# hamaadshah/gan_deeplearning4j

Measured on NVIDIA H100. Metric: images/sec (full G+D step), higher is better.
Workload: dtype bf16

## Files before the change

gan_deeplearning4j_b200/_lib.py:

```python
from __future__ import annotations

import ctypes as C
import os

_HERE = os.path.dirname(os.path.abspath(__file__))
LIB_PATH = os.path.join(_HERE, "lib", "libb200gan.so")
NAME_LEN = 64


class B200GanError(RuntimeError):
    def __init__(self, code, msg):
        super().__init__(f"libb200gan error {code}: {msg}")
        self.code = code


class LayerDesc(C.Structure):
    _fields_ = [("type", C.c_int32), ("name", C.c_char * NAME_LEN), ("n_in", C.c_int32), ("n_out", C.c_int32),
                ("k_h", C.c_int32), ("k_w", C.c_int32), ("s_h", C.c_int32), ("s_w", C.c_int32), ("p_h", C.c_int32), ("p_w", C.c_int32),
                ("has_bias", C.c_int32), ("act", C.c_int32), ("act_alpha", C.c_float), ("updater", C.c_int32),
                ("lr", C.c_float), ("beta1", C.c_float), ("beta2", C.c_float), ("eps", C.c_float), ("l2", C.c_float),
                ("bn_decay", C.c_float), ("bn_eps", C.c_float), ("pre_h", C.c_int32), ("pre_w", C.c_int32), ("pre_c", C.c_int32),
                ("loss", C.c_int32), ("frozen", C.c_int32)]


# ... 25 lines not shown
    _fields_ = [("l1", C.c_float), ("l2", C.c_float), ("l1_bias", C.c_float), ("l2_bias", C.c_float)]


class Constraint(C.Structure):
    _fields_ = [("kind", C.c_int32), ("dims_mask", C.c_int32), ("max_norm", C.c_double), ("min_norm", C.c_double), ("rate", C.c_double)]


class ConvGeom(C.Structure):
    _fields_ = [(k, C.c_int32) for k in ("n", "h", "w", "c", "oh", "ow", "o", "kh", "kw", "sh", "sw", "ph", "pw")]


class TestConvOpts(C.Structure):
    _fields_ = [("epi", C.c_int32), ("act", C.c_int32), ("alpha", C.c_float), ("bias", C.POINTER(C.c_float)), ("scale", C.POINTER(C.c_float)),
                ("groups", C.c_int32), ("aux", C.POINTER(C.c_float)), ("aux2", C.POINTER(C.c_float)), ("stats", C.POINTER(C.c_double)), ("kernel", C.c_char * 64),
                ("bn", C.c_int32), ("max_ctas", C.c_int32), ("poison", C.c_int32), ("w_mn", C.c_int32), ("per_tap", C.c_int32), ("slab", C.c_int32),
                ("defer", C.c_int32), ("db", C.POINTER(C.c_float)), ("param_offset", C.c_int32), ("splits", C.c_int32)]


class EwReduceJob(C.Structure):
    _fields_ = [("n", C.c_int64), ("stride", C.c_int64), ("src_off", C.c_int64), ("dst_off", C.c_int64), ("splits", C.c_int32), ("wide", C.c_int32)]


class TestEwOpts(C.Structure):
    _fields_ = [("op", C.c_int32), ("n", C.c_int64), ("rows", C.c_int32), ("cols", C.c_int32), ("groups", C.c_int32), ("splits", C.c_int32),
                ("stride", C.c_int64)] + [(k, C.c_int32) for k in ("N", "H", "W", "C", "KH", "KW", "SH", "SW", "act")] + [
                ("alpha", C.c_float), ("clip_eps", C.c_float), ("offset", C.c_int32), ("in_place", C.c_int32), ("accumulate", C.c_int32),
                ("poison", C.c_int32), ("n_jobs", C.c_int32), ("jobs", C.POINTER(EwReduceJob)), ("n_seg", C.c_int32),
                ("seg_off", C.POINTER(C.c_int64)), ("seg_len", C.POINTER(C.c_int64)), ("seg_coef", C.POINTER(C.c_float)), ("sumsq", C.c_double),
                ("kernel", C.c_char * 64), ("loss", C.c_int32)]


# ... 107 lines not shown
```

gan_deeplearning4j_b200/csrc/engine.cu:

```cuda
#include <cuda_runtime.h>
#include <dlfcn.h>
#include <math.h>
#include <stdarg.h>
#include <stdio.h>
#include <stdlib.h>
#include <string.h>

#include <algorithm>
#include <string>
#include <vector>

#include "../../include/b200gan.h"
#include "kernels.h"

using namespace b2g;

static thread_local char g_err[1024] = "";
static int32_t fail(int32_t code, const char* fmt, ...) {
  va_list ap; va_start(ap, fmt); vsnprintf(g_err, sizeof(g_err), fmt, ap); va_end(ap); return code;
}
#define CU(call) do { cudaError_t e_ = (call); if (e_ != cudaSuccess) return fail(B2G_ERR_CUDA, "%s:%d %s -> %s", __FILE__, __LINE__, #call, cudaGetErrorString(e_)); } while (0)
#define B2(call) do { int32_t r_ = (call); if (r_ != 0) return r_; } while (0)
#define CHECK_KERNELS() CU(cudaGetLastError())

// ... 1900 lines not shown
    if (!h || prec == PREC_F32) return downF(h, (const float*)d, count);
    float* f = nullptr; B2(upF(nullptr, count, &f)); k_nhwc_to_nchw_f32(prec, d, f, 1, 1, (int)count, s); return downF(h, f, count); }
  int32_t event(cudaEvent_t* e) { CU(cudaEventCreate(e)); events.push_back(*e); return 0; }
};
}

extern "C" int32_t b2g_ctx_allreduce_test(b2g_ctx* c, float* host, int64_t n) {
  if (!c || !host || n < 1) return fail(B2G_ERR_ARG, "null"); if (!c->comm) return fail(B2G_ERR_NCCL, "no communicator"); CU(cudaSetDevice(c->device));
  HookMem m(c->stream, PREC_F32); float* d = nullptr;
  B2(m.upF(host, (size_t)n, &d));
  NC(g_nccl.ar(d, d, (size_t)n, 7, 0, c->comm, c->stream));
  B2(m.downF(host, d, (size_t)n)); CU(cudaStreamSynchronize(c->stream)); return 0;
}

struct TcTestSchedule {
  TcTestSchedule(int bn, int max_ctas, int per_tap, int splits) { g_tc_test_bn = bn; g_tc_test_max_ctas = max_ctas; g_tc_test_per_tap = per_tap; g_tc_test_splits = splits; }
  ~TcTestSchedule() { reset(); }
  void reset() { g_tc_test_bn = 0; g_tc_test_max_ctas = 0; g_tc_test_per_tap = 0; g_tc_test_splits = 0; }
};
enum : unsigned { CO_STATS = 1u << EPI_STATS, CO_BNBWD = 1u << EPI_BNBWD, CO_ACTBWD = 1u << EPI_ACTBWD, CO_BIAS_ACT = 1u << 4, CO_SCALE = 1u << 5,
                  CO_POFF = 1u << 6, CO_BN = 1u << 7, CO_MAX_CTAS = 1u << 8, CO_PER_TAP = 1u << 9, CO_W_MN = 1u << 10, CO_SPLITS = 1u << 11,
                  CO_DEFER = 1u << 12, CO_DB = 1u << 13 };
struct ConvHookImpl {
  const char* kernel;
  bool bf16, tma;
  struct { bool (*shape)(const ConvGeom&); unsigned opts; } kind[3];
};
static bool any_shape(const ConvGeom&) { return true; }
static bool dense_bwd_shape(const ConvGeom& g) { return dense_small_o_supported(g) || dense_small_k_supported(g); }
static bool tc_edge_conv_shape(const ConvGeom& g) { return edge_conv_small_cin_supported(g) && tc_edge_conv_supported(g); }
static bool tc_edge_wgrad_shape(const ConvGeom& g) { return edge_wgrad_small_cin_supported(g) && tc_edge_wgrad_supported(g); }
static const unsigned CO_TC = CO_STATS | CO_BNBWD | CO_ACTBWD | CO_BIAS_ACT | CO_SCALE | CO_BN | CO_MAX_CTAS | CO_PER_TAP;
static const ConvHookImpl kConvHook[6] = {
  {"SIMT kernel", false, false, {{any_shape, CO_BIAS_ACT | CO_SCALE | CO_POFF}, {any_shape, CO_BIAS_ACT | CO_SCALE | CO_POFF}, {any_shape, CO_POFF}}},
  {"tensor-core kernel (BF16, a working tensor-map encoder)", true, true,
   {{tc_fprop_supported, CO_TC | CO_W_MN}, {tc_dgrad_supported, CO_TC}, {tc_wgrad_supported, CO_POFF | CO_SPLITS | CO_DEFER}}},
  {"skinny-layer kernel (<= 4 image channels)", false, false,
   {{edge_conv_small_cin_supported, CO_BIAS_ACT | CO_POFF}, {edge_deconv_small_c_supported, CO_BIAS_ACT | CO_POFF}, {edge_wgrad_small_cin_supported, CO_POFF}}},
  {"skinny-layer tensor-core kernel (BF16, <= 4 image channels, a working tensor-map encoder)", true, true,
   {{tc_edge_conv_shape, CO_BIAS_ACT | CO_MAX_CTAS}, {tc_deconv_ps_supported, CO_ACTBWD | CO_BIAS_ACT | CO_MAX_CTAS},
    {tc_edge_wgrad_shape, CO_POFF | CO_SPLITS | CO_DEFER | CO_DB}}},
  {"dense kernel (1x1 geometry: <= 4 output units, or a short reduction in the input / weight gradient)", false, false,
   {{dense_small_o_supported, CO_BIAS_ACT | CO_POFF}, {dense_bwd_shape, CO_BIAS_ACT | CO_POFF}, {dense_bwd_shape, CO_POFF}}},
  {"few-output conv kernel (BF16, O <= 4, C % 8 == 0, k x k)", true, false,
   {{head_conv_supported, CO_BIAS_ACT | CO_POFF}, {head_conv_supported, CO_BIAS_ACT | CO_POFF}, {head_conv_supported, CO_POFF | CO_SPLITS | CO_DB}}},
};
static constexpr int ik(int impl, int kind) { return 3 * impl + kind; }
// ... 13 lines not shown
    return fail(B2G_ERR_UNSUPPORTED, "impl %d kind %d: no %s for this shape", impl, kind, im.kernel);
  const b2g_test_conv_opts none{}; const b2g_test_conv_opts& o = opt ? *opt : none;
  const struct { unsigned flag; bool set; const char* what; } asked[] = {
    {o.epi >= EPI_STATS && o.epi <= EPI_ACTBWD ? 1u << o.epi : 1u, o.epi != 0,
     "fused epilogue (epi 1-3: the tensor-core fprop / dgrad, impl 1 kind 0 / 1; epi 3: the pixel-shuffle deconv, impl 3 kind 1)"},
    {CO_BIAS_ACT, o.bias || o.act, "bias / activation (kinds 0 / 1; impl 4 kind 1 on its short-reduction kernel)"},
    {CO_SCALE, o.scale != nullptr, "scale (the SIMT and tensor-core fprop / dgrad, impl 0 / 1 kind 0 / 1)"},
    {CO_POFF, o.param_offset != 0, "param_offset (impl 0 / 2 / 4 / 5, and the tensor-core weight gradients, impl 1 / 3 kind 2)"},
    {CO_BN, o.bn != 0, "bn (the tile width of the tensor-core fprop / dgrad, impl 1 kind 0 / 1)"},
    {CO_MAX_CTAS, o.max_ctas != 0, "max_ctas (a grid cap of tc_conv_kernel and tc_edge_conv_kernel launches, impl 1 / 3 kind 0 / 1)"},
    {CO_PER_TAP, o.per_tap != 0, "per_tap (the tensor-core fprop / dgrad, impl 1 kind 0 / 1)"},
    {CO_W_MN, o.w_mn != 0, "w_mn (the [C][O] weight operand of the 1x1 tensor-core fprop, impl 1 kind 0)"},
    {CO_SPLITS, o.splits != 0, "splits (a forced split count of the weight gradients of impl 1 / 3 / 5)"},
    {CO_DEFER, o.defer != 0, "defer (the tensor-core weight gradients, impl 1 / 3 kind 2)"},
    {CO_DB, o.db != nullptr, "db (the bias column of the edge tensor-core and few-output weight gradients, impl 3 / 5 kind 2)"},
  };
  for (const auto& a : asked) if (a.set && !(im.kind[kind].opts & a.flag)) return fail(B2G_ERR_UNSUPPORTED, "impl %d kind %d takes no %s", impl, kind, a.what);
  if (o.param_offset < 0 || o.max_ctas < 0 || o.splits < 0)
    return fail(B2G_ERR_UNSUPPORTED, "param_offset %d, max_ctas %d, splits %d: none may be negative", o.param_offset, o.max_ctas, o.splits);
  if (o.bn && ((o.bn != 64 && o.bn != 128) || oc % o.bn))
    return fail(B2G_ERR_UNSUPPORTED, "bn %d: the tensor-core fprop / dgrad tile is 64 or 128 columns and must divide the %d output channels", o.bn, oc);
  if (impl == 4 && kind == 1 && (o.bias || o.act) && !dense_small_k_supported(g))
    return fail(B2G_ERR_UNSUPPORTED, "impl 4 kind 1: bias / activation run on the short-reduction kernel only, which has no variant for this shape");
  if (o.w_mn && (g.KH != 1 || g.KW != 1)) return fail(B2G_ERR_UNSUPPORTED, "w_mn: the [C][O] weight operand exists for the 1x1 tensor-core fprop only");
  const bool gemm = impl == 0 || impl == 2 || impl >= 4, tc_wg = kind == 2 && (impl == 1 || impl == 3);
  const int force_splits = o.splits;
  size_t sc = std::max(std::max(std::max(k_simt_wgrad_scratch_floats(g), k_tc_wgrad_scratch_floats(g)), std::max(k_edge_wgrad_scratch_floats(g), k_tc_edge_wgrad_scratch_floats(g))), k_dense_small_o_wgrad_scratch_floats(g)) + 16;
  if (force_splits) sc = std::max(sc, (size_t)force_splits * (impl == 1 || impl == 5 ? nw : (size_t)64 * 16 * g.C + 64) + 16);
  if (impl == 5) sc = std::max(sc, std::max(k_head_wgrad_scratch_floats(g), k_colsum_scratch_floats(g.O)) + 16);
  const size_t woff = (prec == PREC_F32 && kind != 2) ? (size_t)o.param_offset : 0, dwoff = kind == 2 ? (size_t)o.param_offset : 0;
// ... 10 lines not shown
  epi.mode = o.epi; epi.scale = scale; epi.imgs_per_group = g.N / groups; epi.act = act; epi.alpha = alpha;
  if (o.epi == EPI_STATS || o.epi == EPI_BNBWD) { B2(m.dev(k_bn_acc_elems(oc, groups), 8, (void**)&d_acc)); epi.acc = d_acc; }
  if (o.epi == EPI_BNBWD || o.epi == EPI_ACTBWD) {
    if (!o.aux) return fail(B2G_ERR_ARG, "epilogue %d needs aux", o.epi);
    void* aux = nullptr; B2(m.upT(o.aux, no, &aux)); epi.aux = (const __nv_bfloat16*)aux;
  }
  if (o.epi == EPI_BNBWD) {
    if (!o.aux2) return fail(B2G_ERR_ARG, "epilogue 2 needs aux2 (the BatchNorm input z)");
    void* aux2 = nullptr; B2(m.upT(o.aux2, no, &aux2)); epi.aux2 = (const __nv_bfloat16*)aux2;
  }
  const TcEpi* pe = o.epi || o.scale ? &epi : nullptr;
  const __nv_bfloat16 *ba = (const __nv_bfloat16*)ta, *bb = (const __nv_bfloat16*)tb; __nv_bfloat16* bo = (__nv_bfloat16*)to;
  ReduceList rl{}; ReduceList* prl = o.defer ? &rl : nullptr;
  cudaEvent_t e0, e1; B2(m.event(&e0)); B2(m.event(&e1));
  int reps = iters < 1 ? 1 : iters; int rc = 0, db_written = 0;
  g_tc_last_kernel = ""; g_tc_last_slab = false; g_tc_last_splits = 0; g_gemm_last_kernel = ""; g_gemm_last_splits = 0;
  TcTestSchedule schedule(o.bn, o.max_ctas, o.per_tap != 0, force_splits);
  for (int it = -1; it < reps; ++it) {
    if (it == 0) CU(cudaEventRecord(e0, s));
    if (d_acc) CU(cudaMemsetAsync(d_acc, 0, 8 * k_bn_acc_elems(oc, groups), s));
    if (o.poison) CU(cudaMemsetAsync(to, 0xFF, ts * no, s));
    if (o.poison && kind == 2) { CU(cudaMemsetAsync(fres, 0xFF, 4 * no, s)); CU(cudaMemsetAsync(scratch, 0xFF, 4 * sc, s)); }
    if (o.poison && dbres) CU(cudaMemsetAsync(dbres, 0xFF, 4 * (size_t)g.O, s));
    switch (ik(impl, kind)) {
      case ik(0, 0): k_simt_fprop(prec, prec, g, ta, tb, bias, to, act, alpha, s, scale); break;
      case ik(0, 1): k_simt_dgrad(prec, prec, g, ta, tb, bias, to, act, alpha, s, scale); break;
      case ik(0, 2): k_simt_wgrad(prec, g, ta, tb, fres, scratch, sc, 0, s); break;
      case ik(1, 0): rc = k_tc_fprop(g, ba, bb, bias, bo, act, alpha, s, pe, o.w_mn ? 1 : 0); break;
      case ik(1, 1): rc = k_tc_dgrad(g, ba, bb, bias, bo, act, alpha, s, pe); break;
      case ik(1, 2): rc = k_tc_wgrad(g, ba, bb, fres, scratch, sc, 0, s, prl); break;
      case ik(2, 0): k_edge_conv_small_cin(prec, prec, g, ta, tb, bias, to, act, alpha, s); break;
      case ik(2, 1): k_edge_deconv_small_c(prec, prec, g, ta, tb, bias, to, act, alpha, s); break;
// ... 19 lines not shown
    }
    if (rc) break;
    if (o.defer) {
      if (!rl.count) { rc = -4; break; }
      k_reduce_multi(rl, s); rl.count = 0;
    }
  }
  schedule.reset();
  CU(cudaEventRecord(e1, s));
  if (rc == -4) return fail(B2G_ERR_CUDA, "defer: the weight gradient queued no reduction");
  if (rc == -5) return fail(B2G_ERR_ARG, "splits %d: the partials do not fit the scratch", force_splits);
  if (rc) return fail(B2G_ERR_CUDA, "tensor-core kernel launch failed (%d)", rc);
  if (opt) {
    strncpy(opt->kernel, gemm ? g_gemm_last_kernel : g_tc_last_kernel, sizeof(opt->kernel) - 1); opt->kernel[sizeof(opt->kernel) - 1] = 0; opt->slab = g_tc_last_slab;
    opt->splits = gemm ? g_gemm_last_splits : tc_wg ? g_tc_last_splits : 0;
  }
  if (o.db) {
    if (!db_written) return fail(B2G_ERR_UNSUPPORTED, "the edge weight gradient produces no bias column for C = %d", g.C);
    B2(m.downF(o.db, dbres, g.O));
  }
  B2(kind == 2 ? m.downF(out, fres, no) : m.downT(out, to, no));
  CU(cudaStreamSynchronize(s)); CHECK_KERNELS();
  if (d_acc && o.stats) {
    std::vector<long long> h(k_bn_acc_elems(oc, groups)); CU(cudaMemcpy(h.data(), d_acc, 8 * h.size(), cudaMemcpyDeviceToHost));
    for (int gi = 0; gi < groups; ++gi) for (int st = 0; st < 2; ++st) for (int ch = 0; ch < oc; ++ch)
      o.stats[((size_t)gi * 2 + st) * oc + ch] = (double)h[((size_t)(gi * 2 + st) * 2 + 0) * oc + ch] / 1024.0 + (double)h[((size_t)(gi * 2 + st) * 2 + 1) * oc + ch] / 1152921504606846976.0;
  }
  float ms = 0.f; CU(cudaEventElapsedTime(&ms, e0, e1)); if (ms_per_iter) *ms_per_iter = ms / reps;
  return 0;
}
// ... 445 lines not shown
```

gan_deeplearning4j_b200/csrc/kernels.h:

```cpp
#pragma once
#include <cuda_runtime.h>
#include <cuda_bf16.h>
#include <math.h>
#include <stdint.h>

namespace b2g {

enum Prec { PREC_F32 = 0, PREC_BF16 = 1 };
enum Act { ACT_IDENTITY = 0, ACT_TANH = 1, ACT_SIGMOID = 2, ACT_RELU = 3, ACT_LRELU = 4,
           ACT_ELU = 5, ACT_SELU = 6, ACT_SOFTPLUS = 7, ACT_SOFTSIGN = 8, ACT_HARDTANH = 9, ACT_HARDSIGMOID = 10, ACT_RELU6 = 11, ACT_SWISH = 12,
           ACT_CUBE = 13, ACT_RATIONALTANH = 14, ACT_RECTIFIEDTANH = 15, ACT_THRESHOLDEDRELU = 16, ACT_EXT_FIRST = ACT_ELU, ACT_EXT_LAST = ACT_THRESHOLDEDRELU };
enum Loss { LOSS_MSE = 2, LOSS_L1 = 3, LOSS_L2 = 4, LOSS_MAE = 5, LOSS_HINGE = 6, LOSS_SQUARED_HINGE = 7, LOSS_WASSERSTEIN = 8 };

inline size_t prec_size(int prec) { return prec == PREC_F32 ? 4 : 2; }

struct ConvGeom {
  int N, H, W, C;
  int OH, OW, O;
  int KH, KW, SH, SW, PH, PW;
};

extern uint64_t g_launch_count;
extern const char* g_ew_last_kernel;
int device_sm_count();
// ... 222 lines not shown
bool head_conv_supported(const ConvGeom& g);
size_t k_head_wgrad_scratch_floats(const ConvGeom& g);
void k_head_fwd(const ConvGeom& g, const __nv_bfloat16* x, const __nv_bfloat16* w, const float* bias, __nv_bfloat16* out, int act, float alpha, cudaStream_t s);
void k_head_dgrad(const ConvGeom& g, const __nv_bfloat16* dy, const __nv_bfloat16* w, const float* bias, __nv_bfloat16* dx, int act, float alpha, cudaStream_t s);
int k_head_wgrad(const ConvGeom& g, const __nv_bfloat16* x, const __nv_bfloat16* dy, float* dw, float* part, size_t part_floats, int force_splits, cudaStream_t s,
                 ReduceList* defer);

bool tc_fprop_supported(const ConvGeom& g);
bool tc_dgrad_supported(const ConvGeom& g);
bool tc_wgrad_supported(const ConvGeom& g);
int  tc_init();
extern const char* g_tc_last_kernel;
extern int g_tc_test_bn, g_tc_test_max_ctas;
extern int g_tc_test_per_tap;
extern bool g_tc_last_slab;
extern int g_tc_test_splits, g_tc_last_splits;
enum { EPI_PLAIN = 0, EPI_STATS = 1, EPI_BNBWD = 2, EPI_ACTBWD = 3 };
struct TcEpi {
  int mode;
  const float* scale;
  unsigned long long* acc;
  int imgs_per_group;
  const __nv_bfloat16* aux;
  const __nv_bfloat16* aux2;
  int act; float alpha;
};
int k_tc_fprop(const ConvGeom& g, const __nv_bfloat16* x, const __nv_bfloat16* w, const float* bias, __nv_bfloat16* out, int act, float alpha, cudaStream_t s, const TcEpi* epi = nullptr, int w_mn = 0);
int k_tc_dgrad(const ConvGeom& g, const __nv_bfloat16* dy, const __nv_bfloat16* w, const float* bias, __nv_bfloat16* dx, int act, float alpha, cudaStream_t s, const TcEpi* epi = nullptr);
int k_tc_wgrad(const ConvGeom& g, const __nv_bfloat16* x, const __nv_bfloat16* dy, float* dw, float* scratch, size_t scratch_floats, int accumulate, cudaStream_t s, ReduceList* defer = nullptr);
size_t k_tc_wgrad_scratch_floats(const ConvGeom& g);
// ... 13 lines not shown
```

gan_deeplearning4j_b200/csrc/kernels_tc.cu:

```cuda
#include <cuda.h>
#include <stdio.h>
#include <stdlib.h>
#include <algorithm>

#include "common.cuh"
#include "kernels.h"

namespace b2g {

typedef CUresult (*PFN_encodeTiled)(CUtensorMap*, CUtensorMapDataType, cuuint32_t, void*, const cuuint64_t*, const cuuint64_t*, const cuuint32_t*,
                                    const cuuint32_t*, CUtensorMapInterleave, CUtensorMapSwizzle, CUtensorMapL2promotion, CUtensorMapFloatOOBfill);
static PFN_encodeTiled g_encode = nullptr;

int tc_init() {
  if (g_encode) return 0;
  void* fn = nullptr; cudaDriverEntryPointQueryResult q;
  if (cudaGetDriverEntryPoint("cuTensorMapEncodeTiled", &fn, cudaEnableDefault, &q) != cudaSuccess || !fn || q != cudaDriverEntryPointSuccess) return -1;
  g_encode = (PFN_encodeTiled)fn; return 0;
}

static int make_map_bf16(CUtensorMap* m, const void* base, int rank, const cuuint64_t* dims, const cuuint64_t* strides_bytes, const cuuint32_t* box, const cuuint32_t* estr) {
  if (!g_encode) return -1;
  CUresult r = g_encode(m, CU_TENSOR_MAP_DATA_TYPE_BFLOAT16, (cuuint32_t)rank, const_cast<void*>(base), dims, strides_bytes, box, estr, CU_TENSOR_MAP_INTERLEAVE_NONE,
                        CU_TENSOR_MAP_SWIZZLE_128B, CU_TENSOR_MAP_L2_PROMOTION_L2_256B, CU_TENSOR_MAP_FLOAT_OOB_FILL_NONE);
// ... 251 lines not shown
        const float s = ((sst[(0 * 2 + st) * BN + col] + sst[(1 * 2 + st) * BN + col]) + sst[(2 * 2 + st) * BN + col]) + sst[(3 * 2 + st) * BN + col];
        sacc_add(p.acc + (size_t)(group * 2 + st) * 2 * p.OC, (size_t)p.OC, (size_t)(nb0 + col), s);
      }
    }
  }
}

template <int BN>
__device__ __forceinline__ void load_b_tile(const TcConvParams& p, const CUtensorMap* tmB, uint32_t dst, uint32_t bar, int ch, int wtap, int nb0) {
  if (!p.b_mn) tma_load_3d(dst, tmB, bar, ch * 64, wtap, nb0);
  else {
#pragma unroll
    for (int j = 0; j < (BN >= 64 ? BN / 64 : 1); ++j) tma_load_3d(dst + j * 8192, tmB, bar, nb0 + j * 64, wtap, ch * 64);
  }
}
template <int BN, int NB, int NACC>
__device__ __forceinline__ void mma_kblock(float (&acc)[NB][NACC], uint32_t a_smem, uint32_t b_smem, int b_mn) {
  const uint64_t adesc = desc_kmajor_sw128(a_smem);
  if constexpr (BN < 64) {
    const uint64_t bdesc = desc_kmajor_sw128(b_smem);
#pragma unroll
    for (int k = 0; k < 4; ++k) wgmma_n16(acc[0], adesc + 2 * k, bdesc + 2 * k);
  } else if constexpr (NB == 2) {
    if (!b_mn) {
#pragma unroll
      for (int k = 0; k < 4; ++k) wgmma_n128<0, 0>(acc[0], acc[1], adesc + 2 * k, desc_kmajor_sw128(b_smem) + 2 * k);
    } else {
#pragma unroll
      for (int k = 0; k < 4; ++k) wgmma_n128<0, 1>(acc[0], acc[1], adesc + 2 * k, desc_mnmajor_sw128(b_smem + k * 2048, 8192));
    }
// ... 7 lines not shown
}
__device__ __forceinline__ void tap_coords(const TcConvParams& p, int ta, int tb, int py, int px, int& ax, int& dy_, int& wtap) {
  if (p.mode == 0) { dy_ = -p.PH + ta; ax = -p.PW + tb; wtap = ta * p.KW + tb; }
  else {
    const int r = py == 0 ? (ta == 0 ? 1 : 3) : (ta == 0 ? 0 : 2), dyr = py == 0 ? (ta == 0 ? 0 : -1) : (ta == 0 ? 1 : 0);
    const int sx = px == 0 ? (tb == 0 ? 1 : 3) : (tb == 0 ? 0 : 2), dxc = px == 0 ? (tb == 0 ? 0 : -1) : (tb == 0 ? 1 : 0);
    dy_ = dyr; ax = dxc; wtap = r * 4 + sx;
  }
}
__device__ __forceinline__ void slab_coords(const TcConvParams& p, int ta, int tb, int py, int px, int& ax, int& dy_, int& wlo, int& whi) {
  int ax2, dy2;
  tap_coords(p, p.mode == 0 ? ta : 1, tb, py, px, ax, dy_, wlo);
  tap_coords(p, p.mode == 0 ? ta + 2 : 0, tb, py, px, ax2, dy2, whi);
}

template <int BN>
struct TcConvRegs {
  static constexpr int LAUNCH = 96, PRODUCER = 24, MMA = BN >= 128 ? 96 : 64, EPI = BN >= 128 ? 128 : 160;
  static_assert(PRODUCER + 2 * MMA + 2 * EPI <= 5 * LAUNCH, "setmaxnreg budget exceeds the launch allocation");
};
template <int BN, int STAGES, int EPI, bool AFFINE, bool PS = false, bool SLAB = false>
__global__ void __launch_bounds__(TC_CONV_THREADS, 1) tc_conv_kernel(const __grid_constant__ CUtensorMap tmA, const __grid_constant__ CUtensorMap tmB, const TcConvParams p) {
  using S = TcSmem<BN, STAGES, EPI, SLAB>;
  using R = TcConvRegs<BN>;
  constexpr int NB = BN >= 64 ? BN / 64 : 1, NACC = BN >= 64 ? 32 : BN / 2;
  extern __shared__ uint8_t smem_raw[];
  const uint32_t smem_base = (smem_u32(smem_raw) + 1023u) & ~1023u;
  uint8_t* smem_gen = smem_raw + (smem_base - smem_u32(smem_raw));
  const uint32_t bar_full = smem_base + S::BAR_OFF;
  const uint32_t bar_empty = bar_full + 8 * STAGES;
  const uint32_t park_full = bar_empty + 8 * STAGES;
  const uint32_t park_empty = park_full + 8 * S::PARKS;
  float* sst = reinterpret_cast<float*>(smem_gen + S::STAT_OFF);
  const int warp = threadIdx.x >> 5, lane = threadIdx.x & 31;
  const int num_kb = p.taps_h * p.taps_w * p.chunks;
  const int tiles = p.tiles_m * p.tiles_n * p.phases;
  auto tile_coords = [&](int t, int& nb0, int& phase, int& n0, int& y0) {
    const int mt = t % p.tiles_m, r = t / p.tiles_m;
    nb0 = (r % p.tiles_n) * BN; phase = r / p.tiles_n;
    if (p.Nt > 1) { n0 = mt * p.Nt; y0 = 0; } else { n0 = mt / p.tiles_y; y0 = (mt % p.tiles_y) * p.Ht; }
  };

  if (threadIdx.x == 0) {
    prefetch_map(&tmA); prefetch_map(&tmB);
    for (int s = 0; s < STAGES; ++s) { mbar_init(bar_full + 8 * s, 1); mbar_init(bar_empty + 8 * s, 8); }
    for (int k = 0; k < S::PARKS; ++k) { mbar_init(park_full + 8 * k, 256); mbar_init(park_empty + 8 * k, 256); }
    fence_mbar_init();
  }
  __syncthreads();
  pdl_wait();

  if (warp >= 16) {
    setmaxnreg_dec<R::PRODUCER>();
    if (warp == 16) {
      int s = 0; uint32_t ph = 0;
      for (int t = blockIdx.x; t < tiles; t += gridDim.x) {
        int nb0, phase, n0, y0; tile_coords(t, nb0, phase, n0, y0);
        const int py = phase >> 1, px = phase & 1;
        const int ybase = p.mode == 0 ? y0 * p.SH : y0;
        int ch = 0, ta = 0, tb = 0;
        int ax, dy_, wtap, wtap2 = 0;
        auto coords = [&]() { if constexpr (SLAB) slab_coords(p, ta, tb, py, px, ax, dy_, wtap, wtap2); else tap_coords(p, ta, tb, py, px, ax, dy_, wtap); };
        coords();
        for (int kb = 0; kb < num_kb; ++kb) {
          mbar_wait(bar_empty + 8 * s, ph ^ 1);
          if (elect_one_sync()) {
            const uint32_t st = smem_base + s * S::STAGE_BYTES;
            mbar_expect_tx(bar_full + 8 * s, SLAB ? p.slab_bytes + S::B_BYTES : S::STAGE_BYTES);
            tma_load_4d(st, &tmA, bar_full + 8 * s, ch * 64, ax, ybase + dy_, n0);
            load_b_tile<BN>(p, &tmB, st + S::A_BYTES, bar_full + 8 * s, ch, wtap, nb0);
            if constexpr (SLAB) load_b_tile<BN>(p, &tmB, st + S::A_BYTES + BN * 128, bar_full + 8 * s, ch, wtap2, nb0);
          }
          __syncwarp();
          if (++s == STAGES) { s = 0; ph ^= 1; }
          if (++ch == p.chunks) { ch = 0; if (++tb == p.taps_w) { tb = 0; ++ta; } coords(); }
        }
      }
    }
  } else if (warp < 8) {
    if constexpr (R::MMA < R::LAUNCH) setmaxnreg_dec<R::MMA>();
    const int wg = warp >> 2;
    const int r0 = wg * 64 + (warp & 3) * 16 + (lane >> 2);
    int s = 0, k = 0; uint32_t ph = 0, kph = 0;
    for (int t = blockIdx.x; t < tiles; t += gridDim.x) {
      float acc[NB][NACC];
#pragma unroll
      for (int nb = 0; nb < NB; ++nb)
#pragma unroll
        for (int j = 0; j < NACC; ++j) acc[nb][j] = 0.f;
      int prev = -1;
      for (int kb = 0; kb < num_kb; ++kb) {
        mbar_wait(bar_full + 8 * s, ph);
// ... 73 lines not shown
        if (p.mode == 0) pix = ((size_t)n * p.outH + gy) * p.outW + gx;
        else pix = ((size_t)n * p.outH + 2 * gy + py) * p.outW + 2 * gx + px;
        const int group = p.imgs_per_group > 0 ? n0 / p.imgs_per_group : 0;
        epi_tile<BN, EPI, AFFINE>(p, srow, pix * p.OC + nb0, nb0, group, sst, reinterpret_cast<uint4*>(smem_gen + S::STG_OFF) + ew * 128, q, lane,
                                  (int)threadIdx.x - 256, half * (BN / 2), (half + 1) * (BN / 2));
        if constexpr (EPI == EPI_STATS || EPI == EPI_BNBWD) epi_bar_sync();
      }
      mbar_arrive(park_empty + 8 * k);
      if (++k == S::PARKS) { k = 0; kph ^= 1; }
    }
  }
}

const char* g_tc_last_kernel = "";
bool g_tc_last_slab = false;
int g_tc_test_bn = 0, g_tc_test_max_ctas = 0, g_tc_test_per_tap = 0, g_tc_test_splits = 0;
int g_tc_last_splits = 0;
static int tc_device() { int dev = 0; cudaGetDevice(&dev); return dev < 0 || dev >= 64 ? 0 : dev; }
#define TC_SET_SMEM_ONCE(kernel, bytes)                                                                                            \
  do { static bool set_[64] = {}; const int d_ = tc_device();                                                                       \
       if (!set_[d_]) { if (cudaFuncSetAttribute(kernel, cudaFuncAttributeMaxDynamicSharedMemorySize, (int)(bytes)) != cudaSuccess) return -2; set_[d_] = true; } } while (0)

static bool pick_row_tile(int N, int GH, int GW, int rows, int* Nt, int* Ht, int* Wt) {
  const int P = GH * GW;
  if (GW > rows || rows % GW) return false;
  if (P >= rows) { if (P % rows) return false; *Nt = 1; *Ht = rows / GW; *Wt = GW; return GH % *Ht == 0; }
  if (rows % P || N % (rows / P)) return false;
  *Nt = rows / P; *Ht = GH; *Wt = GW; return true;
}
static int pick_bn(int OC) { return OC % 128 == 0 ? 128 : OC % 64 == 0 ? 64 : 0; }
static int pick_bn_fill(int OC, long m_tiles_x_phases) {
  if (g_tc_test_bn) return g_tc_test_bn;
  const int target = device_sm_count();
  int bn = pick_bn(OC);
  while (bn > 64 && m_tiles_x_phases * (OC / bn) < target) bn /= 2;
  return bn;
}

bool tc_fprop_supported(const ConvGeom& g) {
  int a, b, c;
  return g.C % 64 == 0 && pick_bn(g.O) != 0 && g.SH >= 1 && g.SH <= 2 && g.SW == g.SH && g.KH * g.KW * (g.C / 64) >= 1 &&
         pick_row_tile(g.N, g.OH, g.OW, 128, &a, &b, &c) && c * g.SW <= 256 && b * g.SH <= 256 && g.N >= 1;
}
bool tc_dgrad_supported(const ConvGeom& g) {
  int a, b, c;
  return g.KH == 4 && g.KW == 4 && g.SH == 2 && g.SW == 2 && g.PH == 1 && g.PW == 1 && g.O % 64 == 0 && pick_bn(g.C) != 0 && g.H == 2 * g.OH && g.W == 2 * g.OW &&
         pick_row_tile(g.N, g.OH, g.OW, 128, &a, &b, &c);
}
static bool tc_epi_ok(const TcEpi* e, int Nt) { return !e || e->mode == EPI_PLAIN || e->mode == EPI_ACTBWD || (e->imgs_per_group > 0 && e->imgs_per_group % Nt == 0 && e->acc); }

template <int BN, int STAGES, int EPI, bool AFFINE, bool PS = false, bool SLAB = false>
static int launch_conv_e(const CUtensorMap& tmA, const CUtensorMap& tmB, const TcConvParams& p, cudaStream_t s) {
  using S = TcSmem<BN, STAGES, EPI, SLAB>;
  TC_SET_SMEM_ONCE((tc_conv_kernel<BN, STAGES, EPI, AFFINE, PS, SLAB>), S::TOTAL);
  const long tiles = (long)p.tiles_m * p.tiles_n * p.phases;
  const unsigned grid = (unsigned)std::min<long>(tiles, g_tc_test_max_ctas > 0 ? g_tc_test_max_ctas : device_sm_count());
  launch_pdl(tc_conv_kernel<BN, STAGES, EPI, AFFINE, PS, SLAB>, dim3(grid), dim3(TC_CONV_THREADS), (size_t)(S::TOTAL), s, tmA, tmB, p);
  LAUNCHED();
  return cudaPeekAtLastError() == cudaSuccess ? 0 : -3;
}
template <int BN, int STAGES, bool SLAB>
static int launch_conv(const CUtensorMap& tmA, const CUtensorMap& tmB, const TcConvParams& p, cudaStream_t s, const char* name) {
  g_tc_last_kernel = name; g_tc_last_slab = SLAB;
  switch (p.epi) {
    case EPI_STATS: return launch_conv_e<BN, STAGES, EPI_STATS, false, false, SLAB>(tmA, tmB, p, s);
    case EPI_BNBWD: return launch_conv_e<BN, STAGES, EPI_BNBWD, false, false, SLAB>(tmA, tmB, p, s);
    case EPI_ACTBWD: return launch_conv_e<BN, STAGES, EPI_ACTBWD, false, false, SLAB>(tmA, tmB, p, s);
  }
  return (p.scale && p.bias) ? launch_conv_e<BN, STAGES, EPI_PLAIN, true, false, SLAB>(tmA, tmB, p, s) : launch_conv_e<BN, STAGES, EPI_PLAIN, false, false, SLAB>(tmA, tmB, p, s);
}
static int dispatch_conv(int BN, bool slab, const CUtensorMap& tmA, const CUtensorMap& tmB, const TcConvParams& p, cudaStream_t s) {
  switch (BN * 2 + slab) {
    case 128: return launch_conv<64, 4, false>(tmA, tmB, p, s, "tc_conv_kernel<64,4>");
    case 256: return launch_conv<128, 4, false>(tmA, tmB, p, s, "tc_conv_kernel<128,4>");
    case 129: return launch_conv<64, 4, true>(tmA, tmB, p, s, "tc_conv_kernel<64,4>");
  }
  return -4;
}
static bool slab_tile(const TcConvParams& p, int BN) {
  if (g_tc_test_per_tap || BN != 64 || p.Wt % 8) return false;
  if (!((p.Nt == 1 && p.Ht >= 2) || (p.Nt == 2 && p.Ht * p.Wt == 64))) return false;
  return p.Nt * (p.Ht + 1) * p.Wt <= SLAB_ROWS;
}
static bool is_k4s2p1_geom(const ConvGeom& g) { return g.KH == 4 && g.KW == 4 && g.SH == 2 && g.SW == 2 && g.PH == 1 && g.PW == 1 && g.H == 2 * g.OH && g.W == 2 * g.OW; }
static void set_slab(TcConvParams& p) {
  p.taps_h = p.mode == 0 ? 2 : 1;
  p.slab_bytes = p.Nt * (p.Ht + 1) * p.Wt * 128;
  p.a_wg_bytes = p.Nt == 1 ? 64 * 128 : (p.Ht + 1) * p.Wt * 128;
  p.a_tap_bytes = p.Wt * 128;
}
// ... 470 lines not shown
```

gan_deeplearning4j_b200/engine.py:

```python
from __future__ import annotations

import copy
import ctypes as C
import math
from typing import Dict, List, Optional, Sequence

import numpy as np

from . import _lib
from ._lib import GanConfig, LayerDesc, LrSchedule, NetConfig, check

LAYER_TYPES = {"conv2d": 0, "deconv2d": 1, "batchnorm": 2, "dense": 3, "activation": 4, "maxpool": 5, "upsample2d": 6,
               "output": 7, "loss": 8, "ff_to_cnn": 9, "cnn_to_ff": 10, "dropout": 11, "subsampling": 12, "global_pooling": 13,
               "cnn_loss": 14, "elementwise": 15, "merge": 16}
ELEMENTWISE_OPS = {"add": 0, "subtract": 1, "product": 2, "average": 3, "max": 4}
VERTEX_TYPES = ("elementwise", "merge")
POOLINGS = {"max": 0, "avg": 1, "sum": 2, "pnorm": 3}
GLOBAL_PNORM_DEFAULT = 2
ACTS = {"identity": 0, "tanh": 1, "sigmoid": 2, "relu": 3, "lrelu": 4, "elu": 5, "selu": 6, "softplus": 7, "softsign": 8, "hardtanh": 9,
        "hardsigmoid": 10, "relu6": 11, "swish": 12, "cube": 13, "rationaltanh": 14, "rectifiedtanh": 15, "thresholdedrelu": 16}
ACT_ALPHA_DEFAULTS = {"elu": 1.0, "thresholdedrelu": 1.0}
LOSSES = {"xent": 0, "mcxent": 1, "mse": 2, "l1": 3, "l2": 4, "mae": 5, "hinge": 6, "squared_hinge": 7, "wasserstein": 8}
UPDATERS = {"sgd": 0, "rmsprop": 1, "adam": 2, "noop": 3, "nesterovs": 4, "adagrad": 5, "adamax": 6, "nadam": 7, "amsgrad": 8, "adadelta": 9}
NO_LR_UPDATERS = ("noop", "adadelta")
# ... 743 lines not shown
def test_conv(ctx: Context, kind: int, impl: int, precision: int, geom: Dict[str, int], a, b, out_size: int, iters: int = 1):
    g = _lib.ConvGeom(**geom)
    a, b = _f32(a).ravel(), _f32(b).ravel()
    out = np.empty(out_size, np.float32)
    ms = C.c_float()
    check(ctx.lib.b2g_test_conv(ctx.h, kind, impl, precision, C.byref(g), _fp(a), _fp(b), _fp(out), iters, C.byref(ms)))
    return out, ms.value


EPI_PLAIN, EPI_STATS, EPI_BNBWD, EPI_ACTBWD = 0, 1, 2, 3


def test_conv_ex(ctx: Context, kind: int, geom: Dict[str, int], a, b, out_size: int, *, epi: int = 0, act: str = "identity", alpha: float = 0.0,
                 bias=None, scale=None, groups: int = 1, aux=None, aux2=None, iters: int = 1, impl: int = 1, bn: int = 0, max_ctas: int = 0,
                 poison: bool = False, w_mn: bool = False, per_tap: bool = False, info: Optional[dict] = None, defer: bool = False, db=None,
                 precision: int = BF16, param_offset: int = 0, splits: int = 0):
    g = _lib.ConvGeom(**geom)
    a, b = _f32(a).ravel(), _f32(b).ravel()
    out = np.empty(out_size, np.float32)
    oc = geom["o"] if kind == 0 else geom["c"]
    o = _lib.TestConvOpts()
    o.epi, o.act, o.alpha, o.groups = epi, ACTS[act], alpha, groups
    o.bn, o.max_ctas, o.poison, o.w_mn, o.per_tap, o.defer = bn, max_ctas, int(poison), int(w_mn), int(per_tap), int(defer)
    o.param_offset, o.splits = param_offset, splits
    if db is not None:
        assert db.dtype == np.float32 and db.flags.c_contiguous
        o.db = _fp(db)
    keep = []
    for name, v in (("bias", bias), ("scale", scale), ("aux", aux), ("aux2", aux2)):
        if v is not None:
            arr = _f32(v).ravel(); keep.append(arr); setattr(o, name, _fp(arr))
    stats = None
    if epi in (EPI_STATS, EPI_BNBWD):
        stats = np.zeros((groups, 2, oc), np.float64); o.stats = stats.ctypes.data_as(C.POINTER(C.c_double))
    ms = C.c_float()
    check(ctx.lib.b2g_test_conv_ex(ctx.h, kind, impl, precision, C.byref(g), _fp(a), _fp(b), _fp(out), iters, C.byref(ms), C.byref(o)))
    if info is not None:
        info["slab"], info["splits"] = bool(o.slab), o.splits
    return out, stats, o.kernel.decode(), ms.value


def test_bn(ctx: Context, precision: int, path: int, x, eps_out, gamma, beta, run_mean, run_var, *, act: str = "identity", alpha: float = 0.0,
            eps: float = 1e-5, decay: float = 0.9, g_gamma=None, g_beta=None, want_param_grads: bool = True):
    x, e = _f32(x), _f32(eps_out)
    groups, rows, ch = x.shape
    par = [_f32(v).ravel() for v in (gamma, beta, run_mean, run_var)]
    r = {k: np.empty(x.shape, np.float32) for k in ("y", "eps_in")}
    r["g_gamma"] = _f32(np.zeros(ch) if g_gamma is None else g_gamma).copy()
    r["g_beta"] = _f32(np.zeros(ch) if g_beta is None else g_beta).copy()
    r.update({k: np.empty(ch, np.float32) for k in ("g_mean", "g_var")})
    r.update({k: np.empty((groups, ch), np.float32) for k in ("mean", "invstd")})
    check(ctx.lib.b2g_test_bn(ctx.h, precision, path, groups, rows, ch, _fp(x), _fp(e), *[_fp(v) for v in par], ACTS[act], alpha, eps, decay,
                              int(want_param_grads), *[_fp(r[k]) for k in ("y", "eps_in", "g_gamma", "g_beta", "g_mean", "g_var", "mean", "invstd")]))
# ... 64 lines not shown
```

include/b200gan.h:

```cpp
#ifndef B200GAN_H
#define B200GAN_H

#include <stddef.h>
#include <stdint.h>

#ifdef __cplusplus
extern "C" {
#endif

#define B2G_VERSION 101
#define B2G_NAME_LEN 64

typedef struct b2g_ctx b2g_ctx;
typedef struct b2g_net b2g_net;
typedef struct b2g_gan b2g_gan;

typedef enum {
  B2G_OK = 0,
  B2G_ERR_ARG = -1,
  B2G_ERR_SHAPE = -2,
  B2G_ERR_CUDA = -3,
  B2G_ERR_NCCL = -4,
  B2G_ERR_OOM = -5,
  B2G_ERR_UNSUPPORTED = -6,
// ... 212 lines not shown
  int32_t act; float alpha;
  const float* bias;
  const float* scale;
  int32_t groups;
  const float* aux;
  const float* aux2;
  double* stats;
  char kernel[64];
  int32_t bn;
  int32_t max_ctas;
  int32_t poison;
  int32_t w_mn;
  int32_t per_tap;
  int32_t slab;
  int32_t defer;
  float* db;
  int32_t param_offset;
  int32_t splits;
} b2g_test_conv_opts;
int32_t b2g_test_conv_ex(b2g_ctx* ctx, int32_t kind, int32_t impl, int32_t precision, const b2g_conv_geom* g,
                         const float* x_or_dy, const float* w_or_x, float* out, int32_t iters, float* ms_per_iter, b2g_test_conv_opts* opts);

int32_t b2g_test_hbm_kernels(b2g_net* net, int32_t rows, int32_t channels, int32_t iters, float* ms3);

int32_t b2g_test_bn(b2g_ctx* ctx, int32_t precision, int32_t path, int32_t groups, int32_t rows, int32_t C, const float* x, const float* eps_out,
                    const float* gamma, const float* beta, const float* run_mean, const float* run_var, int32_t act, float alpha, float eps, float decay,
                    int32_t want_param_grads, float* y, float* eps_in, float* g_gamma, float* g_beta, float* g_mean, float* g_var, float* mean, float* invstd);
int32_t b2g_test_net_shadow(b2g_net* net, int32_t layer, int32_t which, float* out, int64_t n);
int32_t b2g_test_net_noisy_operand(b2g_net* net, int32_t layer, int32_t which, float* out, int64_t n);
int32_t b2g_test_dropout(b2g_ctx* ctx, int32_t precision, uint64_t seed, int32_t layer, int32_t rank, int64_t pass, int32_t rows, int32_t h, int32_t w,
// ... 54 lines not shown
```

Baseline: 92300.

## Add transposed m64n128 wgmma issue path for 64-column slab dgrad tiles

Adds a WT variant of the tensor-core conv kernel for 64-column slab tiles in mode 1 with Nt==1. In this variant each consumer warpgroup processes whole tiles on its own, issuing n128 wgmma with the operands transposed. It gets separate full barriers per warpgroup and a wider register split. The goal is to replace two m64n64 issues per k-step with one wider instruction, making better use of tensor cores. The cost is a doubled barrier set, alternating producer barriers and a new transposed park layout. A test knob (n64) can force the old path.

New measurement: 93380 (median of 6 runs). 1.01x the previous value.

```diff
diff --git a/gan_deeplearning4j_b200/_lib.py b/gan_deeplearning4j_b200/_lib.py
--- a/gan_deeplearning4j_b200/_lib.py
+++ b/gan_deeplearning4j_b200/_lib.py
@@ -63,7 +63,7 @@
     _fields_ = [("epi", C.c_int32), ("act", C.c_int32), ("alpha", C.c_float), ("bias", C.POINTER(C.c_float)), ("scale", C.POINTER(C.c_float)),
                 ("groups", C.c_int32), ("aux", C.POINTER(C.c_float)), ("aux2", C.POINTER(C.c_float)), ("stats", C.POINTER(C.c_double)), ("kernel", C.c_char * 64),
                 ("bn", C.c_int32), ("max_ctas", C.c_int32), ("poison", C.c_int32), ("w_mn", C.c_int32), ("per_tap", C.c_int32), ("slab", C.c_int32),
-                ("defer", C.c_int32), ("db", C.POINTER(C.c_float)), ("param_offset", C.c_int32), ("splits", C.c_int32)]
+                ("defer", C.c_int32), ("n64", C.c_int32), ("db", C.POINTER(C.c_float)), ("param_offset", C.c_int32), ("splits", C.c_int32)]
 
 
 class EwReduceJob(C.Structure):
diff --git a/gan_deeplearning4j_b200/csrc/engine.cu b/gan_deeplearning4j_b200/csrc/engine.cu
--- a/gan_deeplearning4j_b200/csrc/engine.cu
+++ b/gan_deeplearning4j_b200/csrc/engine.cu
@@ -1938,13 +1938,15 @@
 }
 
 struct TcTestSchedule {
-  TcTestSchedule(int bn, int max_ctas, int per_tap, int splits) { g_tc_test_bn = bn; g_tc_test_max_ctas = max_ctas; g_tc_test_per_tap = per_tap; g_tc_test_splits = splits; }
+  TcTestSchedule(int bn, int max_ctas, int per_tap, int splits, int n64) {
+    g_tc_test_bn = bn; g_tc_test_max_ctas = max_ctas; g_tc_test_per_tap = per_tap; g_tc_test_splits = splits; g_tc_test_n64 = n64;
+  }
   ~TcTestSchedule() { reset(); }
-  void reset() { g_tc_test_bn = 0; g_tc_test_max_ctas = 0; g_tc_test_per_tap = 0; g_tc_test_splits = 0; }
+  void reset() { g_tc_test_bn = 0; g_tc_test_max_ctas = 0; g_tc_test_per_tap = 0; g_tc_test_splits = 0; g_tc_test_n64 = 0; }
 };
 enum : unsigned { CO_STATS = 1u << EPI_STATS, CO_BNBWD = 1u << EPI_BNBWD, CO_ACTBWD = 1u << EPI_ACTBWD, CO_BIAS_ACT = 1u << 4, CO_SCALE = 1u << 5,
                   CO_POFF = 1u << 6, CO_BN = 1u << 7, CO_MAX_CTAS = 1u << 8, CO_PER_TAP = 1u << 9, CO_W_MN = 1u << 10, CO_SPLITS = 1u << 11,
-                  CO_DEFER = 1u << 12, CO_DB = 1u << 13 };
+                  CO_DEFER = 1u << 12, CO_DB = 1u << 13, CO_N64 = 1u << 14 };
 struct ConvHookImpl {
   const char* kernel;
   bool bf16, tma;
@@ -1954,7 +1956,7 @@
 static bool dense_bwd_shape(const ConvGeom& g) { return dense_small_o_supported(g) || dense_small_k_supported(g); }
 static bool tc_edge_conv_shape(const ConvGeom& g) { return edge_conv_small_cin_supported(g) && tc_edge_conv_supported(g); }
 static bool tc_edge_wgrad_shape(const ConvGeom& g) { return edge_wgrad_small_cin_supported(g) && tc_edge_wgrad_supported(g); }
-static const unsigned CO_TC = CO_STATS | CO_BNBWD | CO_ACTBWD | CO_BIAS_ACT | CO_SCALE | CO_BN | CO_MAX_CTAS | CO_PER_TAP;
+static const unsigned CO_TC = CO_STATS | CO_BNBWD | CO_ACTBWD | CO_BIAS_ACT | CO_SCALE | CO_BN | CO_MAX_CTAS | CO_PER_TAP | CO_N64;
 static const ConvHookImpl kConvHook[6] = {
   {"SIMT kernel", false, false, {{any_shape, CO_BIAS_ACT | CO_SCALE | CO_POFF}, {any_shape, CO_BIAS_ACT | CO_SCALE | CO_POFF}, {any_shape, CO_POFF}}},
   {"tensor-core kernel (BF16, a working tensor-map encoder)", true, true,
@@ -1998,6 +2000,7 @@
     {CO_SPLITS, o.splits != 0, "splits (a forced split count of the weight gradients of impl 1 / 3 / 5)"},
     {CO_DEFER, o.defer != 0, "defer (the tensor-core weight gradients, impl 1 / 3 kind 2)"},
     {CO_DB, o.db != nullptr, "db (the bias column of the edge tensor-core and few-output weight gradients, impl 3 / 5 kind 2)"},
+    {CO_N64, o.n64 != 0, "n64 (the two-m64n64k16 issue of the tensor-core fprop / dgrad's 64-column tiles, impl 1 kind 0 / 1)"},
   };
   for (const auto& a : asked) if (a.set && !(im.kind[kind].opts & a.flag)) return fail(B2G_ERR_UNSUPPORTED, "impl %d kind %d takes no %s", impl, kind, a.what);
   if (o.param_offset < 0 || o.max_ctas < 0 || o.splits < 0)
@@ -2038,8 +2041,8 @@
   ReduceList rl{}; ReduceList* prl = o.defer ? &rl : nullptr;
   cudaEvent_t e0, e1; B2(m.event(&e0)); B2(m.event(&e1));
   int reps = iters < 1 ? 1 : iters; int rc = 0, db_written = 0;
-  g_tc_last_kernel = ""; g_tc_last_slab = false; g_tc_last_splits = 0; g_gemm_last_kernel = ""; g_gemm_last_splits = 0;
-  TcTestSchedule schedule(o.bn, o.max_ctas, o.per_tap != 0, force_splits);
+  g_tc_last_kernel = ""; g_tc_last_slab = false; g_tc_last_n64 = false; g_tc_last_splits = 0; g_gemm_last_kernel = ""; g_gemm_last_splits = 0;
+  TcTestSchedule schedule(o.bn, o.max_ctas, o.per_tap != 0, force_splits, o.n64 != 0);
   for (int it = -1; it < reps; ++it) {
     if (it == 0) CU(cudaEventRecord(e0, s));
     if (d_acc) CU(cudaMemsetAsync(d_acc, 0, 8 * k_bn_acc_elems(oc, groups), s));
@@ -2089,6 +2092,7 @@
   if (opt) {
     strncpy(opt->kernel, gemm ? g_gemm_last_kernel : g_tc_last_kernel, sizeof(opt->kernel) - 1); opt->kernel[sizeof(opt->kernel) - 1] = 0; opt->slab = g_tc_last_slab;
     opt->splits = gemm ? g_gemm_last_splits : tc_wg ? g_tc_last_splits : 0;
+    opt->n64 = g_tc_last_n64;
   }
   if (o.db) {
     if (!db_written) return fail(B2G_ERR_UNSUPPORTED, "the edge weight gradient produces no bias column for C = %d", g.C);
diff --git a/gan_deeplearning4j_b200/csrc/kernels.h b/gan_deeplearning4j_b200/csrc/kernels.h
--- a/gan_deeplearning4j_b200/csrc/kernels.h
+++ b/gan_deeplearning4j_b200/csrc/kernels.h
@@ -260,6 +260,8 @@
 extern int g_tc_test_bn, g_tc_test_max_ctas;
 extern int g_tc_test_per_tap;
 extern bool g_tc_last_slab;
+extern int g_tc_test_n64;
+extern bool g_tc_last_n64;
 extern int g_tc_test_splits, g_tc_last_splits;
 enum { EPI_PLAIN = 0, EPI_STATS = 1, EPI_BNBWD = 2, EPI_ACTBWD = 3 };
 struct TcEpi {
diff --git a/gan_deeplearning4j_b200/csrc/kernels_tc.cu b/gan_deeplearning4j_b200/csrc/kernels_tc.cu
--- a/gan_deeplearning4j_b200/csrc/kernels_tc.cu
+++ b/gan_deeplearning4j_b200/csrc/kernels_tc.cu
@@ -289,6 +289,11 @@
     for (int j = 0; j < (BN >= 64 ? BN / 64 : 1); ++j) tma_load_3d(dst + j * 8192, tmB, bar, nb0 + j * 64, wtap, ch * 64);
   }
 }
+__device__ __forceinline__ void mma_kblock_wt(float (&acc)[2][32], uint32_t x_smem, uint32_t w_smem) {
+  const uint64_t xdesc = desc_kmajor_sw128(x_smem);
+#pragma unroll
+  for (int k = 0; k < 4; ++k) wgmma_n128<1, 0>(acc[0], acc[1], desc_mnmajor_sw128(w_smem + k * 2048, 8192), xdesc + 2 * k);
+}
 template <int BN, int NB, int NACC>
 __device__ __forceinline__ void mma_kblock(float (&acc)[NB][NACC], uint32_t a_smem, uint32_t b_smem, int b_mn) {
   const uint64_t adesc = desc_kmajor_sw128(a_smem);
@@ -326,21 +331,23 @@
   tap_coords(p, p.mode == 0 ? ta + 2 : 0, tb, py, px, ax2, dy2, whi);
 }
 
-template <int BN>
+template <int BN, bool WT = false>
 struct TcConvRegs {
-  static constexpr int LAUNCH = 96, PRODUCER = 24, MMA = BN >= 128 ? 96 : 64, EPI = BN >= 128 ? 128 : 160;
+  static constexpr bool WIDE = BN >= 128 || WT;
+  static constexpr int LAUNCH = 96, PRODUCER = 24, MMA = WIDE ? 96 : 64, EPI = WIDE ? 128 : 160;
   static_assert(PRODUCER + 2 * MMA + 2 * EPI <= 5 * LAUNCH, "setmaxnreg budget exceeds the launch allocation");
 };
-template <int BN, int STAGES, int EPI, bool AFFINE, bool PS = false, bool SLAB = false>
+template <int BN, int STAGES, int EPI, bool AFFINE, bool PS = false, bool SLAB = false, bool WT = false>
 __global__ void __launch_bounds__(TC_CONV_THREADS, 1) tc_conv_kernel(const __grid_constant__ CUtensorMap tmA, const __grid_constant__ CUtensorMap tmB, const TcConvParams p) {
   using S = TcSmem<BN, STAGES, EPI, SLAB>;
-  using R = TcConvRegs<BN>;
+  using R = TcConvRegs<BN, WT>;
+  static_assert(!WT || (BN == 64 && S::PARKS == 2 && SLAB), "the transposed issue is the 64-column slab tile's, one park slot per consumer warpgroup");
   constexpr int NB = BN >= 64 ? BN / 64 : 1, NACC = BN >= 64 ? 32 : BN / 2;
   extern __shared__ uint8_t smem_raw[];
   const uint32_t smem_base = (smem_u32(smem_raw) + 1023u) & ~1023u;
   uint8_t* smem_gen = smem_raw + (smem_base - smem_u32(smem_raw));
   const uint32_t bar_full = smem_base + S::BAR_OFF;
-  const uint32_t bar_empty = bar_full + 8 * STAGES;
+  const uint32_t bar_empty = bar_full + 8 * STAGES * (WT ? 2 : 1);
   const uint32_t park_full = bar_empty + 8 * STAGES;
   const uint32_t park_empty = park_full + 8 * S::PARKS;
   float* sst = reinterpret_cast<float*>(smem_gen + S::STAT_OFF);
@@ -355,8 +362,9 @@
 
   if (threadIdx.x == 0) {
     prefetch_map(&tmA); prefetch_map(&tmB);
-    for (int s = 0; s < STAGES; ++s) { mbar_init(bar_full + 8 * s, 1); mbar_init(bar_empty + 8 * s, 8); }
-    for (int k = 0; k < S::PARKS; ++k) { mbar_init(park_full + 8 * k, 256); mbar_init(park_empty + 8 * k, 256); }
+    for (int s = 0; s < STAGES; ++s) { mbar_init(bar_full + 8 * s, 1); mbar_init(bar_empty + 8 * s, WT ? 4 : 8); }
+    if constexpr (WT) for (int s = STAGES; s < 2 * STAGES; ++s) mbar_init(bar_full + 8 * s, 1);
+    for (int k = 0; k < S::PARKS; ++k) { mbar_init(park_full + 8 * k, WT ? 128 : 256); mbar_init(park_empty + 8 * k, 256); }
     fence_mbar_init();
   }
   __syncthreads();
@@ -366,6 +374,7 @@
     setmaxnreg_dec<R::PRODUCER>();
     if (warp == 16) {
       int s = 0; uint32_t ph = 0;
+      uint32_t full = bar_full;
       for (int t = blockIdx.x; t < tiles; t += gridDim.x) {
         int nb0, phase, n0, y0; tile_coords(t, nb0, phase, n0, y0);
         const int py = phase >> 1, px = phase & 1;
@@ -378,16 +387,60 @@
           mbar_wait(bar_empty + 8 * s, ph ^ 1);
           if (elect_one_sync()) {
             const uint32_t st = smem_base + s * S::STAGE_BYTES;
-            mbar_expect_tx(bar_full + 8 * s, SLAB ? p.slab_bytes + S::B_BYTES : S::STAGE_BYTES);
-            tma_load_4d(st, &tmA, bar_full + 8 * s, ch * 64, ax, ybase + dy_, n0);
-            load_b_tile<BN>(p, &tmB, st + S::A_BYTES, bar_full + 8 * s, ch, wtap, nb0);
-            if constexpr (SLAB) load_b_tile<BN>(p, &tmB, st + S::A_BYTES + BN * 128, bar_full + 8 * s, ch, wtap2, nb0);
+            mbar_expect_tx(full + 8 * s, SLAB ? p.slab_bytes + S::B_BYTES : S::STAGE_BYTES);
+            tma_load_4d(st, &tmA, full + 8 * s, ch * 64, ax, ybase + dy_, n0);
+            load_b_tile<BN>(p, &tmB, st + S::A_BYTES, full + 8 * s, ch, wtap, nb0);
+            if constexpr (SLAB) load_b_tile<BN>(p, &tmB, st + S::A_BYTES + BN * 128, full + 8 * s, ch, wtap2, nb0);
           }
           __syncwarp();
           if (++s == STAGES) { s = 0; ph ^= 1; }
           if (++ch == p.chunks) { ch = 0; if (++tb == p.taps_w) { tb = 0; ++ta; } coords(); }
         }
+        if constexpr (WT) full = full == bar_full ? bar_full + 8 * STAGES : bar_full;
       }
+    }
+  } else if (warp < 8 && WT) {
+    if constexpr (R::MMA < R::LAUNCH) setmaxnreg_dec<R::MMA>();
+    const int wg = warp >> 2;
+    const uint32_t full = bar_full + wg * 8 * STAGES;
+    float* park = reinterpret_cast<float*>(smem_gen + S::PARK_OFF + wg * S::PARK_BYTES);
+    const int c0 = (warp & 3) * 16 + (lane >> 2), p0 = 2 * (lane & 3);
+    uint32_t g = wg * num_kb;
+    uint32_t fph = 0, kph = 0;
+    for (int t = blockIdx.x + wg * gridDim.x; t < tiles; t += 2 * gridDim.x) {
+      float acc[2][32];
+#pragma unroll
+      for (int nb = 0; nb < 2; ++nb)
+#pragma unroll
+        for (int j = 0; j < 32; ++j) acc[nb][j] = 0.f;
+      int prev = -1;
+      for (int kb = 0; kb < num_kb; ++kb, ++g) {
+        const int s = g % STAGES;
+        mbar_wait(full + 8 * s, (fph >> s) & 1);
+        fph ^= 1u << s;
+        wg_fence();
+        const uint32_t st = smem_base + s * S::STAGE_BYTES;
+        mma_kblock_wt(acc, st, st + S::A_BYTES);
+        mma_kblock_wt(acc, st + p.a_tap_bytes, st + S::A_BYTES + BN * 128);
+        wg_commit();
+        wg_wait<1>();
+        if (prev >= 0 && lane == 0) mbar_arrive(bar_empty + 8 * prev);
+        prev = s;
+      }
+      g += num_kb;
+      wg_wait<0>();
+      if (lane == 0) mbar_arrive(bar_empty + 8 * prev);
+      mbar_wait(park_empty + 8 * wg, kph ^ 1);
+#pragma unroll
+      for (int nb = 0; nb < 2; ++nb)
+#pragma unroll
+        for (int j = 0; j < 8; ++j)
+#pragma unroll
+          for (int i = 0; i < 2; ++i)
+#pragma unroll
+            for (int k = 0; k < 2; ++k) park[(nb * 64 + 8 * j + p0 + k) * S::ACC_PITCH + c0 + 8 * i] = acc[nb][4 * j + 2 * i + k];
+      mbar_arrive(park_full + 8 * wg);
+      kph ^= 1;
     }
   } else if (warp < 8) {
     if constexpr (R::MMA < R::LAUNCH) setmaxnreg_dec<R::MMA>();
@@ -491,7 +544,8 @@
 
 const char* g_tc_last_kernel = "";
 bool g_tc_last_slab = false;
-int g_tc_test_bn = 0, g_tc_test_max_ctas = 0, g_tc_test_per_tap = 0, g_tc_test_splits = 0;
+bool g_tc_last_n64 = false;
+int g_tc_test_bn = 0, g_tc_test_max_ctas = 0, g_tc_test_per_tap = 0, g_tc_test_splits = 0, g_tc_test_n64 = 0;
 int g_tc_last_splits = 0;
 static int tc_device() { int dev = 0; cudaGetDevice(&dev); return dev < 0 || dev >= 64 ? 0 : dev; }
 #define TC_SET_SMEM_ONCE(kernel, bytes)                                                                                            \
@@ -513,6 +567,7 @@
   while (bn > 64 && m_tiles_x_phases * (OC / bn) < target) bn /= 2;
   return bn;
 }
+static bool wt_issue(const TcConvParams& p, int BN, bool slab) { return BN == 64 && slab && p.mode == 1 && p.Nt == 1 && !g_tc_test_n64; }
 
 bool tc_fprop_supported(const ConvGeom& g) {
   int a, b, c;
@@ -526,31 +581,33 @@
 }
 static bool tc_epi_ok(const TcEpi* e, int Nt) { return !e || e->mode == EPI_PLAIN || e->mode == EPI_ACTBWD || (e->imgs_per_group > 0 && e->imgs_per_group % Nt == 0 && e->acc); }
 
-template <int BN, int STAGES, int EPI, bool AFFINE, bool PS = false, bool SLAB = false>
+template <int BN, int STAGES, int EPI, bool AFFINE, bool PS = false, bool SLAB = false, bool WT = false>
 static int launch_conv_e(const CUtensorMap& tmA, const CUtensorMap& tmB, const TcConvParams& p, cudaStream_t s) {
   using S = TcSmem<BN, STAGES, EPI, SLAB>;
-  TC_SET_SMEM_ONCE((tc_conv_kernel<BN, STAGES, EPI, AFFINE, PS, SLAB>), S::TOTAL);
+  TC_SET_SMEM_ONCE((tc_conv_kernel<BN, STAGES, EPI, AFFINE, PS, SLAB, WT>), S::TOTAL);
   const long tiles = (long)p.tiles_m * p.tiles_n * p.phases;
   const unsigned grid = (unsigned)std::min<long>(tiles, g_tc_test_max_ctas > 0 ? g_tc_test_max_ctas : device_sm_count());
-  launch_pdl(tc_conv_kernel<BN, STAGES, EPI, AFFINE, PS, SLAB>, dim3(grid), dim3(TC_CONV_THREADS), (size_t)(S::TOTAL), s, tmA, tmB, p);
+  launch_pdl(tc_conv_kernel<BN, STAGES, EPI, AFFINE, PS, SLAB, WT>, dim3(grid), dim3(TC_CONV_THREADS), (size_t)(S::TOTAL), s, tmA, tmB, p);
   LAUNCHED();
   return cudaPeekAtLastError() == cudaSuccess ? 0 : -3;
 }
-template <int BN, int STAGES, bool SLAB>
+template <int BN, int STAGES, bool SLAB, bool WT = false>
 static int launch_conv(const CUtensorMap& tmA, const CUtensorMap& tmB, const TcConvParams& p, cudaStream_t s, const char* name) {
-  g_tc_last_kernel = name; g_tc_last_slab = SLAB;
+  g_tc_last_kernel = name; g_tc_last_slab = SLAB; g_tc_last_n64 = BN == 64 && !WT;
   switch (p.epi) {
-    case EPI_STATS: return launch_conv_e<BN, STAGES, EPI_STATS, false, false, SLAB>(tmA, tmB, p, s);
-    case EPI_BNBWD: return launch_conv_e<BN, STAGES, EPI_BNBWD, false, false, SLAB>(tmA, tmB, p, s);
-    case EPI_ACTBWD: return launch_conv_e<BN, STAGES, EPI_ACTBWD, false, false, SLAB>(tmA, tmB, p, s);
-  }
-  return (p.scale && p.bias) ? launch_conv_e<BN, STAGES, EPI_PLAIN, true, false, SLAB>(tmA, tmB, p, s) : launch_conv_e<BN, STAGES, EPI_PLAIN, false, false, SLAB>(tmA, tmB, p, s);
+    case EPI_STATS: return launch_conv_e<BN, STAGES, EPI_STATS, false, false, SLAB, WT>(tmA, tmB, p, s);
+    case EPI_BNBWD: return launch_conv_e<BN, STAGES, EPI_BNBWD, false, false, SLAB, WT>(tmA, tmB, p, s);
+    case EPI_ACTBWD: return launch_conv_e<BN, STAGES, EPI_ACTBWD, false, false, SLAB, WT>(tmA, tmB, p, s);
+  }
+  return (p.scale && p.bias) ? launch_conv_e<BN, STAGES, EPI_PLAIN, true, false, SLAB, WT>(tmA, tmB, p, s) : launch_conv_e<BN, STAGES, EPI_PLAIN, false, false, SLAB, WT>(tmA, tmB, p, s);
 }
 static int dispatch_conv(int BN, bool slab, const CUtensorMap& tmA, const CUtensorMap& tmB, const TcConvParams& p, cudaStream_t s) {
-  switch (BN * 2 + slab) {
-    case 128: return launch_conv<64, 4, false>(tmA, tmB, p, s, "tc_conv_kernel<64,4>");
-    case 256: return launch_conv<128, 4, false>(tmA, tmB, p, s, "tc_conv_kernel<128,4>");
-    case 129: return launch_conv<64, 4, true>(tmA, tmB, p, s, "tc_conv_kernel<64,4>");
+  const bool wt = wt_issue(p, BN, slab);
+  switch (BN * 4 + wt * 2 + slab) {
+    case 256: return launch_conv<64, 4, false>(tmA, tmB, p, s, "tc_conv_kernel<64,4>");
+    case 257: return launch_conv<64, 4, true>(tmA, tmB, p, s, "tc_conv_kernel<64,4>");
+    case 259: return launch_conv<64, 4, true, true>(tmA, tmB, p, s, "tc_conv_kernel<64,4>");
+    case 512: return launch_conv<128, 4, false>(tmA, tmB, p, s, "tc_conv_kernel<128,4>");
   }
   return -4;
 }
diff --git a/gan_deeplearning4j_b200/engine.py b/gan_deeplearning4j_b200/engine.py
--- a/gan_deeplearning4j_b200/engine.py
+++ b/gan_deeplearning4j_b200/engine.py
@@ -781,7 +781,7 @@
 def test_conv_ex(ctx: Context, kind: int, geom: Dict[str, int], a, b, out_size: int, *, epi: int = 0, act: str = "identity", alpha: float = 0.0,
                  bias=None, scale=None, groups: int = 1, aux=None, aux2=None, iters: int = 1, impl: int = 1, bn: int = 0, max_ctas: int = 0,
                  poison: bool = False, w_mn: bool = False, per_tap: bool = False, info: Optional[dict] = None, defer: bool = False, db=None,
-                 precision: int = BF16, param_offset: int = 0, splits: int = 0):
+                 precision: int = BF16, param_offset: int = 0, splits: int = 0, n64: bool = False):
     g = _lib.ConvGeom(**geom)
     a, b = _f32(a).ravel(), _f32(b).ravel()
     out = np.empty(out_size, np.float32)
@@ -789,7 +789,7 @@
     o = _lib.TestConvOpts()
     o.epi, o.act, o.alpha, o.groups = epi, ACTS[act], alpha, groups
     o.bn, o.max_ctas, o.poison, o.w_mn, o.per_tap, o.defer = bn, max_ctas, int(poison), int(w_mn), int(per_tap), int(defer)
-    o.param_offset, o.splits = param_offset, splits
+    o.param_offset, o.splits, o.n64 = param_offset, splits, int(n64)
     if db is not None:
         assert db.dtype == np.float32 and db.flags.c_contiguous
         o.db = _fp(db)
@@ -803,7 +803,7 @@
     ms = C.c_float()
     check(ctx.lib.b2g_test_conv_ex(ctx.h, kind, impl, precision, C.byref(g), _fp(a), _fp(b), _fp(out), iters, C.byref(ms), C.byref(o)))
     if info is not None:
-        info["slab"], info["splits"] = bool(o.slab), o.splits
+        info["slab"], info["n64"], info["splits"] = bool(o.slab), bool(o.n64), o.splits
     return out, stats, o.kernel.decode(), ms.value
 
 
diff --git a/include/b200gan.h b/include/b200gan.h
--- a/include/b200gan.h
+++ b/include/b200gan.h
@@ -250,6 +250,7 @@
   int32_t per_tap;
   int32_t slab;
   int32_t defer;
+  int32_t n64;
   float* db;
   int32_t param_offset;
   int32_t splits;
```
